# bbye98/mdhelper

Hardware: AMD Instinct MI355X
Metric: pair-distances binned/sec (higher is better)
Workload: dtype f32 filter + f64 contract arithmetic, u64 counts

## Files before the change

mdhelper_amd/csrc/mdx_rdf.hip:

```cpp

#include "mdx_common.hpp"
#include "mdx_internal.hpp"
#include "mdx_molecules.hpp"
#include "mdx_rdf_device.hpp"
#include "mdx_rdf_cell.hpp"
#include "mdx_traj.hpp"

#include <cmath>

namespace mdx {


static double thresh_ge(double e)
{
    if (!(e > 0.0))
        return 0.0;
    double t = e * e;
    while (std::sqrt(t) >= e && t > 0.0)
        t = std::nextafter(t, 0.0);
    while (std::sqrt(t) < e)
        t = std::nextafter(t, INFINITY);
    return t;
}

// ... 392 lines not shown
        if (!lazy_orig)
            MDX_TRY(h->d_po2.ensure(16 * e_p2));
        MDX_TRY(h->d_bb2.ensure(16 * e_b2));
    }
    unsigned *d_misc = h->d_misc.as<unsigned>();
    if (!tri)
        hipLaunchKernelGGL(rdf_check_boxes_kernel, dim3((unsigned)ceil_div(n_frames, 256)), dim3(256),
                           0, h->stream, d_boxes, n_frames, d_misc + 1);

    size_t base = sizeof(float4) * 256 + sizeof(double) * (h->n_bins + 1);
    const size_t lds_budget = 64 * 1024;
    const size_t lds_six_blocks = 13 * 1024;
    int n_hist = 8;
    while (n_hist > 4 && base + size_t(n_hist) * cell_hist_stride(h->n_bins) * 4 > lds_six_blocks)
        n_hist >>= 1;
    while (n_hist > 1 && base + size_t(n_hist) * cell_hist_stride(h->n_bins) * 4 > lds_budget)
        n_hist >>= 1;
    size_t lds = base + size_t(n_hist) * cell_hist_stride(h->n_bins) * 4;
    const bool gh = lds > lds_budget;
    if (gh)
        lds = sizeof(float4) * 256;
    const bool lower = h->edges.front() > 0.0;
    void (*kern)(CellArgs) = nullptr;
#define MDX_CELL_PICK(E, L)                                                                     \
    kern = tri ? (gh ? rdf_cell_pair_kernel<E, L, 1, true> : rdf_cell_pair_kernel<E, L, 0, true>) \
               : (gh ? rdf_cell_pair_kernel<E, L, 1> : rdf_cell_pair_kernel<E, L, 0>)
    if (excl && lower) MDX_CELL_PICK(true, true);
    else if (excl) MDX_CELL_PICK(true, false);
    else if (lower) MDX_CELL_PICK(false, true);
    else MDX_CELL_PICK(false, false);
#undef MDX_CELL_PICK
    if (h->occ_kernel != reinterpret_cast<const void *>(kern) || h->occ_lds != lds) {
        int per_cu = 0, cus = 0;
        MDX_HIP(hipOccupancyMaxActiveBlocksPerMultiprocessor(&per_cu, reinterpret_cast<const void *>(kern), 256, lds));
        MDX_HIP(hipDeviceGetAttribute(&cus, hipDeviceAttributeMultiprocessorCount, h->dev));
        h->occ_kernel = reinterpret_cast<const void *>(kern);
        h->occ_lds = lds;
        h->occ_blocks_per_xcd = std::max<int64_t>(1, int64_t(std::max(per_cu, 1)) * std::max(cus, 8) / 8);
    }
    const int64_t blocks_per_xcd = h->occ_blocks_per_xcd;

    hipStream_t s_sort = h->stream;
    for (int64_t f0 = 0; f0 < n_frames; f0 += slab) {
        const int64_t nf = std::min(slab, n_frames - f0);
        float4 *pw1 = h->d_pw1.as<float4>();
        float4 *po1 = lazy_orig ? nullptr : h->d_po1.as<float4>();
        float4 *bb1 = h->d_bb1.as<float4>(), *bc1 = h->d_bb16_1.as<float4>();
        float4 *pw2 = self ? pw1 : h->d_pw2.as<float4>();
        float4 *po2 = self ? po1 : (lazy_orig ? nullptr : h->d_po2.as<float4>());
// ... 796 lines not shown
```

mdhelper_amd/csrc/mdx_rdf_cell.hpp:

```cpp
#pragma once

#include "mdx_rdf_device.hpp"

struct CellArgs {
    const float4 *pw1, *po1, *bb1;
    const float4 *pw2, *po2, *bb2;
    const float4 *bb16_2;
    const float *in1, *in2;
    int n1_in, n2_in;
    const float *boxes;
    const float *tri;
    const double *thresh;
    unsigned long long *counts;
    const unsigned *maxabs_bits;
    unsigned long long *exact_counter;
    unsigned long long *tilepair_counter;
    unsigned long long *clock_counter;
    double t_lo, t_hi, r0, r1;
    int n1p, n2p;
    int n_bins, n_hist, n_rep;
    int self, frame0;
    int n_frames;
    int tags_everywhere;
    unsigned *work;
    unsigned flush_units;
    int spread;
};

constexpr unsigned CELL_WORK_STRIDE = 32;
constexpr size_t CELL_WORK_BYTES = 8 * CELL_WORK_STRIDE * 4;

constexpr int CELL_MAX = 16384;
constexpr int SORT_THREADS = 1024;
constexpr int CELL_QCAP = 1024;
constexpr int CELL_CHUNK = 1;
constexpr int CELL_NCHUNK = 64 / CELL_CHUNK;
constexpr int CELL_TODO = 128;
__host__ __device__ constexpr int cell_hist_stride(int n_bins) { return n_bins + 1; }

struct HistLdsRep {
    unsigned *h;
    int sh;
    __device__ inline void add(int k, unsigned w) const { atomicAdd(h + (k << sh), w); }
};
__device__ inline int cell_hist_shift(const HistLdsRep &h) { return h.sh; }
template <typename Hist> __device__ inline int cell_hist_shift(const Hist &) { return 0; }

struct CellGrid {
    int nc[3];
    float Lf[3];
    double Ld[3], invLd[3];
    __device__ inline void init(const float *box, int n)
    {
        double vol = 1.0;
#pragma unroll
        for (int k = 0; k < 3; ++k) {
            Lf[k] = box[k];
            Ld[k] = (double)box[k];
            invLd[k] = 1.0 / Ld[k];
            vol *= Ld[k];
        }
        const double a = cbrt(64.0 * vol / (double)max(n, 1));
        nc[0] = min(max((int)rint(Ld[0] / a), 1), 64);
        nc[1] = min(max((int)rint(Ld[1] / a), 1), 64);
        nc[2] = max((int)rint(16.0 * Ld[2] / a), 1);
        while (nc[0] * nc[1] * nc[2] > CELL_MAX)
// ... 258 lines not shown
};

__device__ inline float cell_uniform(float v)
{
    return __int_as_float(__builtin_amdgcn_readfirstlane(__float_as_int(v)));
}

__device__ inline const __constant__ CellArgs *cell_args()
{
    auto p = __builtin_amdgcn_kernarg_segment_ptr();
    asm volatile("" : "+s"(p));
    return (const __constant__ CellArgs *)p;
}

__device__ inline unsigned cell_opaque(unsigned v)
{
    v = __builtin_amdgcn_readfirstlane(v);
    asm volatile("" : "+s"(v));
    return v;
}

struct CellWave {
    uint2 *todo;
    unsigned n_todo;
    unsigned overflow;
    unsigned n_exact;
};

template <bool LOWER, int TAGS>
__device__ inline void cell_filter(const CellHot &c, float fx, float fy, float fz, int tag_i,
                                   int tag_j, float &pos, bool &cand, bool &sure)
{
    float r2 = __fmaf_rn(fz, fz, __fmaf_rn(fy, fy, fx * fx));
    pos = __fmaf_rn(__builtin_amdgcn_sqrtf(r2), c.inv_w, c.pos0);
    const float t = __builtin_amdgcn_fractf(pos);
    cand = LOWER ? (r2 < c.cand_hi && r2 >= c.cand_lo) : (r2 < c.cand_hi);
    sure = t < c.sure_w;
    if (TAGS)
        cand = cand && (tag_i != tag_j);
}

__device__ inline void cell_exact_ctx(const CellHot &c, const CellArgs &a, PairCtx<true> &cx)
{
#pragma unroll
    for (int k = 0; k < 3; ++k) {
        cx.Ld[k] = (double)c.L[k];
        cx.invd[k] = (double)c.invL[k];
    }
    cx.r0f = (float)a.r0;
    cx.inv_wf = c.inv_w;
}

template <bool LOWER, int TAGS, int MODE, typename Hist>
__device__ inline void cell_step(const CellHot &c, const CellArgs &a, const Hist &hist, float fx,
                                 float fy, float fz, int tag_i, int tag_j, unsigned i_base,
                                 unsigned j_idx, unsigned w, CellWave &wv)
{
    float r2 = __fmaf_rn(fz, fz, __fmaf_rn(fy, fy, fx * fx));
    const float pos = __fmaf_rn(__builtin_amdgcn_sqrtf(r2), c.inv_w, c.pos0);
    const float t = __builtin_amdgcn_fractf(pos);
    unsigned long long m_todo;
    if (MODE == 1) {
        bool cand = LOWER ? (r2 < c.cand_hi && r2 >= c.cand_lo) : (r2 < c.cand_hi);
        if (TAGS)
            cand = cand && (tag_i != tag_j);
        const bool sure = t < c.sure_w;
        m_todo = __builtin_amdgcn_ballot_w64(cand && !sure);
        if (cand && sure && pos < (float)a.n_bins)
            hist.add((int)pos, w);
    } else {
        const unsigned hbase = (unsigned)(size_t)(__attribute__((address_space(3))) unsigned *)hist.h;
        const int hshift = cell_hist_shift(hist) + 2;
        unsigned tmp;
        if (LOWER && TAGS)
            asm volatile("v_cmpx_gt_f32_e32 %[hi], %[r2]\n\tv_cmpx_le_f32_e32 %[lo], %[r2]\n\tv_cmpx_ne_u32_e32 %[ti], %[tj]\n\t"
                         "v_cmp_le_f32_e64 %[mt], %[sw], %[t]\n\tv_cvt_i32_f32_e32 %[tmp], %[pos]\n\t"
                         "s_andn2_b64 exec, exec, %[mt]\n\tv_lshl_add_u32 %[tmp], %[tmp], %[sh], %[hb]\n\t"
                         "ds_add_u32 %[tmp], %[w]\n\ts_mov_b64 exec, -1"
                         : [mt] "=&s"(m_todo), [tmp] "=&v"(tmp)
                         : [hi] "s"(c.cand_hi), [lo] "s"(c.cand_lo), [r2] "v"(r2), [sw] "s"(c.sure_w), [t] "v"(t),
                           [pos] "v"(pos), [hb] "v"(hbase), [w] "v"(w), [sh] "s"(hshift), [ti] "v"(tag_i), [tj] "v"(tag_j)
                         : "memory");
        else if (LOWER)
            asm volatile("v_cmpx_gt_f32_e32 %[hi], %[r2]\n\tv_cmpx_le_f32_e32 %[lo], %[r2]\n\t"
                         "v_cmp_le_f32_e64 %[mt], %[sw], %[t]\n\tv_cvt_i32_f32_e32 %[tmp], %[pos]\n\t"
                         "s_andn2_b64 exec, exec, %[mt]\n\tv_lshl_add_u32 %[tmp], %[tmp], %[sh], %[hb]\n\t"
                         "ds_add_u32 %[tmp], %[w]\n\ts_mov_b64 exec, -1"
                         : [mt] "=&s"(m_todo), [tmp] "=&v"(tmp)
                         : [hi] "s"(c.cand_hi), [lo] "s"(c.cand_lo), [r2] "v"(r2), [sw] "s"(c.sure_w), [t] "v"(t),
                           [pos] "v"(pos), [hb] "v"(hbase), [w] "v"(w), [sh] "s"(hshift)
                         : "memory");
        else if (TAGS)
            asm volatile("v_cmpx_gt_f32_e32 %[hi], %[r2]\n\tv_cmpx_ne_u32_e32 %[ti], %[tj]\n\t"
                         "v_cmp_le_f32_e64 %[mt], %[sw], %[t]\n\tv_cvt_i32_f32_e32 %[tmp], %[pos]\n\t"
                         "s_andn2_b64 exec, exec, %[mt]\n\tv_lshl_add_u32 %[tmp], %[tmp], %[sh], %[hb]\n\t"
                         "ds_add_u32 %[tmp], %[w]\n\ts_mov_b64 exec, -1"
                         : [mt] "=&s"(m_todo), [tmp] "=&v"(tmp)
                         : [hi] "s"(c.cand_hi), [r2] "v"(r2), [sw] "s"(c.sure_w), [t] "v"(t), [pos] "v"(pos),
                           [hb] "v"(hbase), [w] "v"(w), [sh] "s"(hshift), [ti] "v"(tag_i), [tj] "v"(tag_j)
                         : "memory");
        else
            asm volatile("v_cmpx_gt_f32_e32 %[hi], %[r2]\n\t"
                         "v_cmp_le_f32_e64 %[mt], %[sw], %[t]\n\tv_cvt_i32_f32_e32 %[tmp], %[pos]\n\t"
                         "s_andn2_b64 exec, exec, %[mt]\n\tv_lshl_add_u32 %[tmp], %[tmp], %[sh], %[hb]\n\t"
                         "ds_add_u32 %[tmp], %[w]\n\ts_mov_b64 exec, -1"
                         : [mt] "=&s"(m_todo), [tmp] "=&v"(tmp)
                         : [hi] "s"(c.cand_hi), [r2] "v"(r2), [sw] "s"(c.sure_w), [t] "v"(t), [pos] "v"(pos),
                           [hb] "v"(hbase), [w] "v"(w), [sh] "s"(hshift)
                         : "memory");
    }
    if (__builtin_expect(m_todo != 0ull, 0)) {
        const unsigned cnt = (unsigned)__popcll(m_todo);
        if (wv.n_todo + cnt <= (unsigned)CELL_TODO) {
            if ((m_todo >> (threadIdx.x & 63u)) & 1ull) {
                const unsigned rank = __builtin_amdgcn_mbcnt_hi(
                    (unsigned)(m_todo >> 32), __builtin_amdgcn_mbcnt_lo((unsigned)m_todo, 0u));
                wv.todo[wv.n_todo + rank] =
                    make_uint2(i_base + (threadIdx.x & 63u), j_idx);
            }
            wv.n_todo += cnt;
        } else {
            wv.overflow = 1u;
        }
    }
}

template <typename Hist>
__device__ inline void cell_flush(const CellHot &c, const CellArgs &a, const double *sT,
                                  const Hist &hist, CellWave &wv, const CellOrig &po1f,
                                  const CellOrig &po2f)
{
    __builtin_amdgcn_fence(__ATOMIC_RELEASE, "wavefront");
    __builtin_amdgcn_wave_barrier();
    __builtin_amdgcn_fence(__ATOMIC_ACQUIRE, "wavefront");
    PairCtx<true> cx;
    cell_exact_ctx(c, a, cx);
    const unsigned lane = threadIdx.x & 63u;
    for (unsigned e0 = 0; e0 < wv.n_todo; e0 += 64u) {
        if (e0 + lane < wv.n_todo) {
            const uint2 e = wv.todo[e0 + lane];
            cell_pair_exact(cx, a, sT, hist, po1f.at(e.x), po2f.at(e.y & 0x7fffffffu),
                            (e.y >> 31) + 1u, c.tri);
        }
    }
    wv.n_exact += wv.n_todo;
    wv.n_todo = 0u;
    __builtin_amdgcn_fence(__ATOMIC_RELEASE, "wavefront");
    __builtin_amdgcn_wave_barrier();
}

template <bool LOWER, bool EXCL, typename Hist>
__device__ inline void cell_slow_unit(const CellHot &c, const CellArgs &a, const double *sT,
                                      const Hist &hist, const float4 *sJw, int j0, int nj,
                                      unsigned u_mask, bool tags, int general, const float *geo,
                                      const float4 &p0, const float4 &p1, const CellOrig &po1f,
                                      const CellOrig &po2f, unsigned i_idx0, unsigned jbase,
                                      unsigned w, CellWave &wv)
{
    for (int jj = j0; jj < j0 + nj; ++jj) {
        const float4 q = sJw[jj];
        for (int u = 0; u < 2; ++u) {
            if (!((u_mask >> u) & 1u))
                continue;
            const float4 &p = u ? p1 : p0;
            float fx = q.x - p.x, fy = q.y - p.y, fz = q.z - p.z;
            if (general & 1)
                fx = fminf(fabsf(fx), c.L[0] - fabsf(fx));
            if (general & 2)
                fy = fminf(fabsf(fy), c.L[1] - fabsf(fy));
            if (general & 4)
                fz = fminf(fabsf(fz), c.L[2] - fabsf(fz));
            float pos;
            bool cand, sure;
            cell_filter<LOWER, 0>(c, fx, fy, fz, 0, 0, pos, cand, sure);
            if (EXCL && tags)
                cand = cand && (__float_as_int(p.w) != __float_as_int(q.w));
            const bool todo = cand && !sure;
            const unsigned long long m_todo = __builtin_amdgcn_ballot_w64(todo);
            if (m_todo == 0ull)
                continue;
            if (wv.n_todo > (unsigned)CELL_TODO - 64u)
                cell_flush(c, a, sT, hist, wv, po1f, po2f);
            if (todo) {
                const unsigned rank = __builtin_amdgcn_mbcnt_hi(
                    (unsigned)(m_todo >> 32), __builtin_amdgcn_mbcnt_lo((unsigned)m_todo, 0u));
                wv.todo[wv.n_todo + rank] =
                    make_uint2(i_idx0 + 64u * u, (jbase + jj) | ((w - 1u) << 31));
            }
            wv.n_todo += (unsigned)__popcll(m_todo);
        }
    }
}

template <bool EXCL, bool LOWER, int MODE, bool TRI = false>
__global__ __launch_bounds__(256, TRI ? 4 : 7) void rdf_cell_pair_kernel(CellArgs a)
{
    constexpr bool GH = MODE == 1;
    extern __shared__ __align__(16) unsigned char smem_raw[];
    float4 *sJ = reinterpret_cast<float4 *>(smem_raw);
    double *sT = reinterpret_cast<double *>(smem_raw + sizeof(float4) * 256);
    unsigned *sh = reinterpret_cast<unsigned *>(sT + (a.n_bins + 1));
    __shared__ unsigned s_exact, s_units, s_general, s_qn, s_qnext, s_next;
    __shared__ unsigned sQ[CELL_QCAP];
    __shared__ uint2 s_todo[4][CELL_TODO];
    __shared__ float s_geo[48];
    __shared__ unsigned sQimg[TRI ? CELL_QCAP : 1];

    const int tid = threadIdx.x, lane = tid & 63, wave = tid >> 6;
    long long clk0 = 0, rt0 = 0;
    if (a.clock_counter && tid == 0) {
        clk0 = clock64();
        rt0 = wall_clock64();
    }
    const int t64_2 = a.n2p / 64;

    if (!GH) {
        for (int b = tid; b <= a.n_bins; b += 256)
            sT[b] = a.thresh[b];
        for (int b = tid; b < a.n_hist * cell_hist_stride(a.n_bins); b += 256)
            sh[b] = 0u;
    }
    if (tid == 0) {
        s_exact = 0u;
        s_units = 0u;
        s_general = 0u;
        s_next = atomicAdd(a.work + CELL_WORK_STRIDE * (blockIdx.x & 7u), 1u);
    }
    __syncthreads();

    unsigned long long *out = a.counts + int64_t(blockIdx.x % unsigned(a.n_rep)) * a.n_bins;
    const double *thr = GH ? a.thresh : sT;
    const int rep_log = __builtin_amdgcn_readfirstlane(31 - __clz(a.n_hist));
    HistLdsRep hl{sh + (GH ? 0 : (lane & (a.n_hist - 1))), GH ? 0 : rep_log};
    HistGlobal hg{out};
    CellHot hot{};

    float4 *sJw = sJ + wave * 64;
    CellWave wv{s_todo[wave], 0u, 0u, 0u};
    unsigned n_units = 0, n_general = 0;
    unsigned lds_units = 0;
    for (;;) {
    const unsigned item = __builtin_amdgcn_readfirstlane(s_next);
    int frame_l, I;
    {
        const unsigned xcd = cell_opaque(blockIdx.x) & 7u;
        const auto *A = cell_args();
        const unsigned tiles = unsigned(A->n1p) >> 7;
        if (A->spread) {
            const unsigned g = item * 8u + xcd;
            if (g >= unsigned(A->n_frames) * tiles)
                break;
            const unsigned fq = __builtin_amdgcn_readfirstlane(g / tiles);
            frame_l = int(fq);
            I = int(g - fq * tiles);
        } else {
            const unsigned nfx = unsigned(A->n_frames + 7 - int(xcd)) >> 3;
            if (item >= nfx * tiles)
                break;
            const unsigned fq = __builtin_amdgcn_readfirstlane(item / tiles);
            frame_l = int(fq * 8u + xcd);
            I = int(item - fq * tiles);
// ... 21 lines not shown
            PairCtx<true> ctx;
            if (TRI) {
                const float *B = A->tri + int64_t(frame) * 9;
                float sum = 0.f;
                for (int i = 0; i < 9; ++i) {
                    s_geo[31 + i] = B[i];
                    sum += fabsf(B[i]);
                }
                const float pseudo[3] = {4.f * sum, 4.f * sum, 4.f * sum};
                ctx.init(pseudo, A->maxabs_bits, A->r0, A->r1, A->n_bins);
            } else {
                ctx.init(A->boxes + int64_t(frame) * 6, A->maxabs_bits, A->r0, A->r1, A->n_bins);
            }
            const float Lmax = fmaxf(ctx.Lf[0], fmaxf(ctx.Lf[1], ctx.Lf[2]));
            const float cut = sqrtf(ctx.cand_hi) + 1e-5f * Lmax;
            for (int k = 0; k < 3; ++k) {
                s_geo[k] = ctx.Lf[k];
                s_geo[3 + k] = ctx.invf[k];
            }
            s_geo[6] = cut;
            s_geo[7] = cut * cut;
            s_geo[26] = ctx.cand_hi;
            s_geo[27] = ctx.cand_lo;
            s_geo[28] = ctx.inv_wf;
            s_geo[29] = -ctx.r0f * ctx.inv_wf - ctx.eta;
            s_geo[30] = 1.0f - 2.0f * ctx.eta;
        }
        const float4 *BB1 = A->bb1 + int64_t(frame) * (A->n1p / 64) * 2 + int64_t(I) * 4;
        const float4 l0 = BB1[0], h0 = BB1[1], l1 = BB1[2], h1 = BB1[3];
        const float lo0[3] = {l0.x, l0.y, l0.z}, hi0[3] = {h0.x, h0.y, h0.z};
        const float lo1[3] = {l1.x, l1.y, l1.z}, hi1[3] = {h1.x, h1.y, h1.z};
        for (int k = 0; k < 3; ++k) {
            const float lo = fminf(lo0[k], lo1[k]), hi = fmaxf(hi0[k], hi1[k]);
            s_geo[8 + k] = 0.5f * (lo + hi);
            s_geo[11 + k] = 0.5f * (hi - lo);
            s_geo[14 + k] = 0.5f * (lo0[k] + hi0[k]);
            s_geo[17 + k] = 0.5f * (lo1[k] + hi1[k]);
            s_geo[20 + k] = 0.5f * (hi0[k] - lo0[k]);
            s_geo[23 + k] = 0.5f * (hi1[k] - lo1[k]);
        }
        s_qn = 0u;
        s_qnext = 0u;
    }
    float4 p0, p1;
    {
        const auto *A = cell_args();
        const float4 *PW1 = A->pw1 + int64_t(frame) * A->n1p + int64_t(I) * 128;
        int l = lane;
        asm volatile("" : "+v"(l));
// ... 176 lines not shown
                    const float hJ[3] = {0.5f * (hi.x - lo.x), 0.5f * (hi.y - lo.y), 0.5f * (hi.z - lo.z)};
                    sg2 = 0.f;
#pragma unroll
                    for (int k = 0; k < 3; ++k) {
                        float gap = fmaxf(0.f, fabsf(cJ[k] - s_geo[14 + 3 * h + k]) -
                                                   (s_geo[20 + 3 * h + k] + hJ[k]));
                        sg2 = __fmaf_rn(gap, gap, sg2);
                    }
                }
                sub = __ballot(sg2 <= s_geo[7]) & SUB_ALL;
            }
            __builtin_amdgcn_fence(__ATOMIC_RELEASE, "wavefront");
            sJw[lane] = pj;
            __builtin_amdgcn_fence(__ATOMIC_ACQUIRE, "wavefront");
            __builtin_amdgcn_wave_barrier();
            const bool diag = a.self && Jt <= 2 * I + 1;
            unsigned w = (a.self && !diag) ? 2u : 1u;
            asm volatile("" : "+v"(w));
            const unsigned jbase = unsigned(Jt) * 64u | ((a.self && !diag) ? 0x80000000u : 0u);
            const bool tags = EXCL && (a.tags_everywhere || diag);
            if (!gen) {
                const unsigned mark = wv.n_todo;
                n_units += (unsigned)__popcll(sub) + (CELL_CHUNK == 1 ? (unsigned)__popcll(sub1) : 0u);
#define MDX_CELL_HALF(TG, P, IB, Q, JJ)                                                            \
    if (GH) cell_step<LOWER, TG, MODE>(hot, a, hg, Q.x - P.x, Q.y - P.y, Q.z - P.z, __float_as_int(P.w), __float_as_int(Q.w), IB, (JJ), w, wv); \
    else cell_step<LOWER, TG, MODE>(hot, a, hl, Q.x - P.x, Q.y - P.y, Q.z - P.z, __float_as_int(P.w), __float_as_int(Q.w), IB, (JJ), w, wv);
#define MDX_CELL_UNITS_CHUNKS(TG)                                                                         \
    for (unsigned long long rem = sub; rem;) {                                                     \
        const int s = __builtin_ctzll(rem) >> 1;                                                   \
        const unsigned bits = unsigned(rem >> (2 * s)) & 3u;                                       \
        rem &= ~(3ull << (2 * s));                                                                 \
        const unsigned jg = jbase + unsigned(CELL_CHUNK * s);                                      \
        float4 q[CELL_CHUNK];                                                                      \
        _Pragma("unroll") for (int c = 0; c < CELL_CHUNK; ++c) q[c] = sJw[CELL_CHUNK * s + c];     \
               \
        if (CELL_CHUNK == 2) asm volatile("" ::"v"(q[0].w), "v"(q[1].w));                          \
        else _Pragma("unroll") for (int c = 0; c < CELL_CHUNK; ++c) asm volatile("" ::"v"(q[c].w)); \
        if (bits & 1u) {                                                                           \
            _Pragma("unroll") for (int c = 0; c < CELL_CHUNK; ++c)                                 \
            {                                                                                      \
                MDX_CELL_HALF(TG, p0, i_base0, q[c], jg + unsigned(c))                             \
            }                                                                                      \
        }                                                                                          \
        if (bits & 2u) {                                                                           \
            _Pragma("unroll") for (int c = 0; c < CELL_CHUNK; ++c)                                 \
            {                                                                                      \
                MDX_CELL_HALF(TG, p1, i_base0 + 64u, q[c], jg + unsigned(c))                       \
            }                                                                                      \
        }                                                                                          \
    }
#define MDX_CELL_ROW_LOOP(TG, MASK, BODY)                                                          \
    for (unsigned long long rem = (MASK); rem;) {                                                  \
        const int r = __builtin_ctzll(rem);                                                        \
        asm("s_bitset0_b64 %0, %1" : "+s"(rem) : "s"(r));                                          \
        const float4 q = sJw[r];                                                                   \
        asm volatile("" ::"v"(q.w));                                       \
        BODY                                                                                       \
    }
#define MDX_CELL_ROW2_LOOP(TG, MASK, BODY)                                                         \
    for (unsigned long long rem = (MASK); rem;) {                                                  \
        const int r = __builtin_ctzll(rem);                                                        \
        asm("s_bitset0_b64 %0, %1" : "+s"(rem) : "s"(r));                                          \
        const float4 q = sJw[r], q1 = sJw[r + 1];                                                  \
        asm volatile("" ::"v"(q.w), "v"(q1.w));                                                    \
        BODY                                                                                       \
    }
#define MDX_CELL_UNITS_ROWS(TG)                                                                    \
    {                                                                                              \
        const unsigned long long both = sub & sub1;                                                \
         \
        const unsigned long long pairs = both & (both >> 1) & 0x5555555555555555ull;               \
        const unsigned long long paired = pairs | (pairs << 1);                                    \
        MDX_CELL_ROW2_LOOP(TG, pairs,                                                              \
                          MDX_CELL_HALF(TG, p0, i_base0, q, jbase + unsigned(r))                   \
                          MDX_CELL_HALF(TG, p0, i_base0, q1, jbase + unsigned(r) + 1u)             \
                          MDX_CELL_HALF(TG, p1, i_base0 + 64u, q, jbase + unsigned(r))             \
                          MDX_CELL_HALF(TG, p1, i_base0 + 64u, q1, jbase + unsigned(r) + 1u))      \
        MDX_CELL_ROW_LOOP(TG, both & ~paired,                                                      \
                          MDX_CELL_HALF(TG, p0, i_base0, q, jbase + unsigned(r))                   \
                          MDX_CELL_HALF(TG, p1, i_base0 + 64u, q, jbase + unsigned(r)))            \
                                                  \
        const unsigned long long only0 = sub & ~sub1, only1 = sub1 & ~sub;                         \
        const unsigned long long pairs0 = only0 & (only0 >> 1) & 0x5555555555555555ull;            \
        const unsigned long long pairs1 = only1 & (only1 >> 1) & 0x5555555555555555ull;            \
        MDX_CELL_ROW2_LOOP(TG, pairs0,                                                             \
                          MDX_CELL_HALF(TG, p0, i_base0, q, jbase + unsigned(r))                   \
                          MDX_CELL_HALF(TG, p0, i_base0, q1, jbase + unsigned(r) + 1u))            \
        MDX_CELL_ROW2_LOOP(TG, pairs1,                                                             \
                          MDX_CELL_HALF(TG, p1, i_base0 + 64u, q, jbase + unsigned(r))             \
                          MDX_CELL_HALF(TG, p1, i_base0 + 64u, q1, jbase + unsigned(r) + 1u))      \
        MDX_CELL_ROW_LOOP(TG, only0 & ~(pairs0 | (pairs0 << 1)),                                   \
                          MDX_CELL_HALF(TG, p0, i_base0, q, jbase + unsigned(r)))                  \
        MDX_CELL_ROW_LOOP(TG, only1 & ~(pairs1 | (pairs1 << 1)),                                   \
                          MDX_CELL_HALF(TG, p1, i_base0 + 64u, q, jbase + unsigned(r)))            \
    }
#define MDX_CELL_UNITS(TG)                                                                         \
    if (CELL_CHUNK == 1) {                                                                         \
        MDX_CELL_UNITS_ROWS(TG)                                                                    \
    } else {                                                                                       \
        MDX_CELL_UNITS_CHUNKS(TG)                                                                  \
    }
                if (tags) {
                    MDX_CELL_UNITS(1)
                } else {
                    MDX_CELL_UNITS(0)
                }
#undef MDX_CELL_UNITS
#undef MDX_CELL_UNITS_ROWS
#undef MDX_CELL_ROW_LOOP
#undef MDX_CELL_ROW2_LOOP
#undef MDX_CELL_UNITS_CHUNKS
#undef MDX_CELL_HALF
                if (__builtin_expect(wv.overflow != 0u, 0)) {
                    wv.overflow = 0u;
                    wv.n_todo = mark;
                    for (unsigned long long rem = CELL_CHUNK == 1 ? (sub | sub1) : sub; rem;) {
                        const int s = CELL_CHUNK == 1 ? __builtin_ctzll(rem) : (__builtin_ctzll(rem) >> 1);
                        const unsigned bits = CELL_CHUNK == 1
                                                  ? (unsigned((sub >> s) & 1ull) | (unsigned((sub1 >> s) & 1ull) << 1))
                                                  : (unsigned(rem >> (2 * s)) & 3u);
                        rem &= CELL_CHUNK == 1 ? ~(1ull << s) : ~(3ull << (2 * s));
                        if (GH) cell_slow_unit<LOWER, EXCL>(hot, a, thr, hg, sJw, CELL_CHUNK * s, CELL_CHUNK, bits, tags, 0, s_geo, p0, p1, MDX_PO1F(), MDX_PO2(), i_idx0, jbase, w, wv);
                        else cell_slow_unit<LOWER, EXCL>(hot, a, thr, hl, sJw, CELL_CHUNK * s, CELL_CHUNK, bits, tags, 0, s_geo, p0, p1, MDX_PO1F(), MDX_PO2(), i_idx0, jbase, w, wv);
                    }
                }
            } else {
                n_units += 2 * CELL_NCHUNK;
                n_general += 2 * CELL_NCHUNK;
                const unsigned mark = wv.n_todo;
#define MDX_CELL_GENERAL(GM)                                                                       \
    _Pragma("unroll 2") for (int jj = 0; jj < 64; ++jj)                                            \
    {                                                                                              \
        float4 q = sJw[jj];                                                                        \
        asm volatile("" ::"v"(q.w));  \
        _Pragma("unroll") for (int u = 0; u < 2; ++u)                                              \
        {                                                                                          \
            const float4 &p = u ? p1 : p0;                                                         \
            float fx = q.x - p.x, fy = q.y - p.y, fz = q.z - p.z;                                  \
            if ((GM) & 1) fx = fminf(fabsf(fx), hot.L[0] - fabsf(fx));                             \
            if ((GM) & 2) fy = fminf(fabsf(fy), hot.L[1] - fabsf(fy));                             \
            if ((GM) & 4) fz = fminf(fabsf(fz), hot.L[2] - fabsf(fz));                             \
            if (GH) cell_step<LOWER, EXCL ? 1 : 0, MODE>(hot, a, hg, fx, fy, fz, __float_as_int(p.w), __float_as_int(q.w), i_base0 + 64u * u, jbase + jj, w, wv); \
            else cell_step<LOWER, EXCL ? 1 : 0, MODE>(hot, a, hl, fx, fy, fz, __float_as_int(p.w), __float_as_int(q.w), i_base0 + 64u * u, jbase + jj, w, wv); \
        }                                                                                          \
    }
                switch (gen) {
                case 1: MDX_CELL_GENERAL(1) break;
                case 2: MDX_CELL_GENERAL(2) break;
                case 3: MDX_CELL_GENERAL(3) break;
                case 4: MDX_CELL_GENERAL(4) break;
                case 5: MDX_CELL_GENERAL(5) break;
                case 6: MDX_CELL_GENERAL(6) break;
                default: MDX_CELL_GENERAL(7) break;
                }
#undef MDX_CELL_GENERAL
                if (__builtin_expect(wv.overflow != 0u, 0)) {
                    wv.overflow = 0u;
                    wv.n_todo = mark;
                    if (GH) cell_slow_unit<LOWER, EXCL>(hot, a, thr, hg, sJw, 0, 64, 3u, true, gen, s_geo, p0, p1, MDX_PO1F(), MDX_PO2(), i_idx0, jbase, w, wv);
                    else cell_slow_unit<LOWER, EXCL>(hot, a, thr, hl, sJw, 0, 64, 3u, true, gen, s_geo, p0, p1, MDX_PO1F(), MDX_PO2(), i_idx0, jbase, w, wv);
                }
            }
            if (wv.n_todo >= 64u) {
                if (GH) cell_flush(hot, a, thr, hg, wv, MDX_PO1F(), MDX_PO2());
                else cell_flush(hot, a, thr, hl, wv, MDX_PO1F(), MDX_PO2());
            }
            }
        }
        if (round0 + CELL_QCAP >= t64_2 && wv.n_todo) {
            if (GH) cell_flush(hot, a, thr, hg, wv, MDX_PO1F(), MDX_PO2());
            else cell_flush(hot, a, thr, hl, wv, MDX_PO1F(), MDX_PO2());
        }
        __syncthreads();
    }
    }
#undef MDX_PO1F
#undef MDX_PO2
    }
    if (lane == 0) {
        if (wv.n_exact) atomicAdd(&s_exact, wv.n_exact);
        if (n_units) atomicAdd(&s_units, n_units);
        if (n_general) atomicAdd(&s_general, n_general);
    }
    __syncthreads();
    if (tid == 0) {
        const unsigned so = rdf_stat_offset(blockIdx.x);
        if (s_exact) atomicAdd(a.exact_counter + so, (unsigned long long)s_exact);
        if (s_units) atomicAdd(a.tilepair_counter + so, (unsigned long long)s_units);
        if (s_general) atomicAdd(a.tilepair_counter + so + 1, (unsigned long long)s_general);
        if (a.clock_counter) {
            atomicAdd(a.clock_counter + so, (unsigned long long)(clock64() - clk0));
            atomicAdd(a.clock_counter + so + 1, (unsigned long long)(wall_clock64() - rt0));
        }
    }
// ... 11 lines not shown
```

Measured before the change: 2118 billion.

## Add fixed-point bin mode and move todo-queue append into inline asm slow path

Adds a MODE==2 kernel variant, used when LDS histograms are used and there are at most 254 bins. It scales the bin position by 2^16 and converts it to u32, so the integer bin is the high 16 bits and the fractional 'sure' test becomes a 16-bit integer compare. This replaces fract plus float compare with cvt_u32, cmp_u16 and mad_u32_u16, with a bias applied to the histogram base. The todo-queue append for ambiguous pairs also moves into the inline asm as an out-of-line subsection branch, which removes the ballot and popcount C++ path from the hot loop. Both changes aim to cut VALU and SALU instructions per pair, at the cost of more complex asm and some precision-handling risk near bin edges.

```diff
diff --git a/mdhelper_amd/csrc/mdx_rdf.hip b/mdhelper_amd/csrc/mdx_rdf.hip
--- a/mdhelper_amd/csrc/mdx_rdf.hip
+++ b/mdhelper_amd/csrc/mdx_rdf.hip
@@ -438,9 +438,14 @@
         lds = sizeof(float4) * 256;
     const bool lower = h->edges.front() > 0.0;
     void (*kern)(CellArgs) = nullptr;
+    bool fxp = !gh && h->n_bins + 2 <= 256;
+    if (const char *e = getenv("MDX_RDF_CELL_FIXED"))
+        fxp = fxp && atoi(e) != 0;
 #define MDX_CELL_PICK(E, L)                                                                     \
-    kern = tri ? (gh ? rdf_cell_pair_kernel<E, L, 1, true> : rdf_cell_pair_kernel<E, L, 0, true>) \
-               : (gh ? rdf_cell_pair_kernel<E, L, 1> : rdf_cell_pair_kernel<E, L, 0>)
+    kern = tri ? (gh ? rdf_cell_pair_kernel<E, L, 1, true>                                      \
+                     : fxp ? rdf_cell_pair_kernel<E, L, 2, true> : rdf_cell_pair_kernel<E, L, 0, true>) \
+               : (gh ? rdf_cell_pair_kernel<E, L, 1>                                            \
+                     : fxp ? rdf_cell_pair_kernel<E, L, 2> : rdf_cell_pair_kernel<E, L, 0>)
     if (excl && lower) MDX_CELL_PICK(true, true);
     else if (excl) MDX_CELL_PICK(true, false);
     else if (lower) MDX_CELL_PICK(false, true);
diff --git a/mdhelper_amd/csrc/mdx_rdf_cell.hpp b/mdhelper_amd/csrc/mdx_rdf_cell.hpp
--- a/mdhelper_amd/csrc/mdx_rdf_cell.hpp
+++ b/mdhelper_amd/csrc/mdx_rdf_cell.hpp
@@ -41,7 +41,8 @@
 struct HistLdsRep {
     unsigned *h;
     int sh;
-    __device__ inline void add(int k, unsigned w) const { atomicAdd(h + (k << sh), w); }
+    int bias;
+    __device__ inline void add(int k, unsigned w) const { atomicAdd(h + ((k + bias) << sh), w); }
 };
 __device__ inline int cell_hist_shift(const HistLdsRep &h) { return h.sh; }
 template <typename Hist> __device__ inline int cell_hist_shift(const Hist &) { return 0; }
@@ -346,24 +347,35 @@
 
 struct CellWave {
     uint2 *todo;
+    unsigned todo_lds;
     unsigned n_todo;
     unsigned overflow;
     unsigned n_exact;
 };
 
-template <bool LOWER, int TAGS>
+__device__ inline unsigned cell_fx_u32(float P)
+{
+    unsigned u;
+    asm("v_cvt_u32_f32_e32 %0, %1" : "=v"(u) : "v"(P));
+    return u;
+}
+
+template <bool LOWER, int TAGS, bool FX>
 __device__ inline void cell_filter(const CellHot &c, float fx, float fy, float fz, int tag_i,
-                                   int tag_j, float &pos, bool &cand, bool &sure)
+                                   int tag_j, bool &cand, bool &sure)
 {
     float r2 = __fmaf_rn(fz, fz, __fmaf_rn(fy, fy, fx * fx));
-    pos = __fmaf_rn(__builtin_amdgcn_sqrtf(r2), c.inv_w, c.pos0);
-    const float t = __builtin_amdgcn_fractf(pos);
+    const float pos = __fmaf_rn(__builtin_amdgcn_sqrtf(r2), c.inv_w, c.pos0);
     cand = LOWER ? (r2 < c.cand_hi && r2 >= c.cand_lo) : (r2 < c.cand_hi);
-    sure = t < c.sure_w;
+    if (FX)
+        sure = (cell_fx_u32(pos) & 0xffffu) < __float_as_uint(c.sure_w);
+    else
+        sure = __builtin_amdgcn_fractf(pos) < c.sure_w;
     if (TAGS)
         cand = cand && (tag_i != tag_j);
 }
 
+template <bool FX>
 __device__ inline void cell_exact_ctx(const CellHot &c, const CellArgs &a, PairCtx<true> &cx)
 {
 #pragma unroll
@@ -372,84 +384,98 @@
         cx.invd[k] = (double)c.invL[k];
     }
     cx.r0f = (float)a.r0;
-    cx.inv_wf = c.inv_w;
-}
-
-template <bool LOWER, int TAGS, int MODE, typename Hist>
+    cx.inv_wf = FX ? c.inv_w * 0x1p-16f : c.inv_w;
+}
+
+#define MDX_STEP_PRE_00 "v_cmpx_gt_f32_e32 %[hi], %[r2]\n\t"
+#define MDX_STEP_PRE_10 MDX_STEP_PRE_00 "v_cmpx_le_f32_e32 %[lo], %[r2]\n\t"
+#define MDX_STEP_PRE_01 MDX_STEP_PRE_00 "v_cmpx_ne_u32_e32 %[ti], %[tj]\n\t"
+#define MDX_STEP_PRE_11 MDX_STEP_PRE_10 "v_cmpx_ne_u32_e32 %[ti], %[tj]\n\t"
+#define MDX_STEP_BIN_FLOAT                                                                         \
+    "v_cmp_le_f32_e32 vcc, %[sw], %[y]\n\tv_cvt_i32_f32_e32 %[tmp], %[x]\n\t"                      \
+    "s_andn2_b64 exec, exec, vcc\n\tv_lshl_add_u32 %[tmp], %[tmp], %[sh], %[hb]\n\t"
+#define MDX_STEP_BIN_FX                                                                            \
+    "v_cvt_u32_f32_e32 %[y], %[x]\n\tv_cmp_le_u16_e32 vcc, %[sw], %[y]\n\t"                        \
+    "v_mad_u32_u16 %[tmp], %[y], %[sh], %[hb] op_sel:[1,0,0,0]\n\ts_andn2_b64 exec, exec, vcc\n\t"
+#define MDX_STEP_TAIL                                                                              \
+    "ds_add_u32 %[tmp], %[w]\n\ts_mov_b64 exec, -1\n\ts_cbranch_vccnz .Lmdx_todo_%=\n"             \
+    ".Lmdx_back_%=:\n\t.subsection 1\n"                                                            \
+    ".Lmdx_todo_%=:\n\ts_bcnt1_i32_b64 %[st], vcc\n\ts_add_u32 %[st], %[st], %[nt]\n\t"            \
+    "s_cmp_gt_u32 %[st], %[cap]\n\ts_cbranch_scc1 .Lmdx_full_%=\n\t"                               \
+    "v_mbcnt_lo_u32_b32 %[y], vcc_lo, 0\n\tv_mbcnt_hi_u32_b32 %[y], vcc_hi, %[y]\n\t"              \
+    "v_add_u32_e32 %[y], %[nt], %[y]\n\tv_lshl_add_u32 %[y], %[y], 3, %[td]\n\t"                   \
+    "v_mbcnt_lo_u32_b32 %[tmp], -1, 0\n\tv_mbcnt_hi_u32_b32 %[tmp], -1, %[tmp]\n\t"                \
+    "v_add_u32_e32 %[tmp], %[ib], %[tmp]\n\tv_mov_b32_e32 %[x], %[jb]\n\t"                         \
+    "v_add_u32_e32 %[x], %[jr], %[x]\n\tv_add_u32_e32 %[x], %[jo], %[x]\n\t"                       \
+    "s_mov_b64 exec, vcc\n\tds_write2_b32 %[y], %[tmp], %[x] offset1:1\n\t"                        \
+    "s_mov_b64 exec, -1\n\ts_mov_b32 %[nt], %[st]\n\ts_branch .Lmdx_back_%=\n"                     \
+    ".Lmdx_full_%=:\n\ts_mov_b32 %[ov], 1\n\ts_branch .Lmdx_back_%=\n\t.subsection 0\n\t"
+template <bool LOWER, int TAGS, int MODE, int JO = 0, typename Hist>
 __device__ inline void cell_step(const CellHot &c, const CellArgs &a, const Hist &hist, float fx,
                                  float fy, float fz, int tag_i, int tag_j, unsigned i_base,
-                                 unsigned j_idx, unsigned w, CellWave &wv)
+                                 unsigned jbase, unsigned jr, unsigned w, CellWave &wv)
 {
     float r2 = __fmaf_rn(fz, fz, __fmaf_rn(fy, fy, fx * fx));
-    const float pos = __fmaf_rn(__builtin_amdgcn_sqrtf(r2), c.inv_w, c.pos0);
-    const float t = __builtin_amdgcn_fractf(pos);
-    unsigned long long m_todo;
+    float pos = __fmaf_rn(__builtin_amdgcn_sqrtf(r2), c.inv_w, c.pos0);
     if (MODE == 1) {
+        const float t = __builtin_amdgcn_fractf(pos);
         bool cand = LOWER ? (r2 < c.cand_hi && r2 >= c.cand_lo) : (r2 < c.cand_hi);
         if (TAGS)
             cand = cand && (tag_i != tag_j);
         const bool sure = t < c.sure_w;
-        m_todo = __builtin_amdgcn_ballot_w64(cand && !sure);
+        const unsigned long long m_todo = __builtin_amdgcn_ballot_w64(cand && !sure);
         if (cand && sure && pos < (float)a.n_bins)
             hist.add((int)pos, w);
+        if (__builtin_expect(m_todo != 0ull, 0)) {
+            const unsigned cnt = (unsigned)__popcll(m_todo);
+            if (wv.n_todo + cnt <= (unsigned)CELL_TODO) {
+                if ((m_todo >> (threadIdx.x & 63u)) & 1ull) {
+                    const unsigned rank = __builtin_amdgcn_mbcnt_hi(
+                        (unsigned)(m_todo >> 32), __builtin_amdgcn_mbcnt_lo((unsigned)m_todo, 0u));
+                    wv.todo[wv.n_todo + rank] = make_uint2(i_base + (threadIdx.x & 63u), jbase + jr + unsigned(JO));
+                }
+                wv.n_todo += cnt;
+            } else {
+                wv.overflow = 1u;
+            }
+        }
     } else {
+        constexpr bool FX = MODE == 2;
         const unsigned hbase = (unsigned)(size_t)(__attribute__((address_space(3))) unsigned *)hist.h;
-        const int hshift = cell_hist_shift(hist) + 2;
-        unsigned tmp;
-        if (LOWER && TAGS)
-            asm volatile("v_cmpx_gt_f32_e32 %[hi], %[r2]\n\tv_cmpx_le_f32_e32 %[lo], %[r2]\n\tv_cmpx_ne_u32_e32 %[ti], %[tj]\n\t"
-                         "v_cmp_le_f32_e64 %[mt], %[sw], %[t]\n\tv_cvt_i32_f32_e32 %[tmp], %[pos]\n\t"
-                         "s_andn2_b64 exec, exec, %[mt]\n\tv_lshl_add_u32 %[tmp], %[tmp], %[sh], %[hb]\n\t"
-                         "ds_add_u32 %[tmp], %[w]\n\ts_mov_b64 exec, -1"
-                         : [mt] "=&s"(m_todo), [tmp] "=&v"(tmp)
-                         : [hi] "s"(c.cand_hi), [lo] "s"(c.cand_lo), [r2] "v"(r2), [sw] "s"(c.sure_w), [t] "v"(t),
-                           [pos] "v"(pos), [hb] "v"(hbase), [w] "v"(w), [sh] "s"(hshift), [ti] "v"(tag_i), [tj] "v"(tag_j)
-                         : "memory");
-        else if (LOWER)
-            asm volatile("v_cmpx_gt_f32_e32 %[hi], %[r2]\n\tv_cmpx_le_f32_e32 %[lo], %[r2]\n\t"
-                         "v_cmp_le_f32_e64 %[mt], %[sw], %[t]\n\tv_cvt_i32_f32_e32 %[tmp], %[pos]\n\t"
-                         "s_andn2_b64 exec, exec, %[mt]\n\tv_lshl_add_u32 %[tmp], %[tmp], %[sh], %[hb]\n\t"
-                         "ds_add_u32 %[tmp], %[w]\n\ts_mov_b64 exec, -1"
-                         : [mt] "=&s"(m_todo), [tmp] "=&v"(tmp)
-                         : [hi] "s"(c.cand_hi), [lo] "s"(c.cand_lo), [r2] "v"(r2), [sw] "s"(c.sure_w), [t] "v"(t),
-                           [pos] "v"(pos), [hb] "v"(hbase), [w] "v"(w), [sh] "s"(hshift)
-                         : "memory");
-        else if (TAGS)
-            asm volatile("v_cmpx_gt_f32_e32 %[hi], %[r2]\n\tv_cmpx_ne_u32_e32 %[ti], %[tj]\n\t"
-                         "v_cmp_le_f32_e64 %[mt], %[sw], %[t]\n\tv_cvt_i32_f32_e32 %[tmp], %[pos]\n\t"
-                         "s_andn2_b64 exec, exec, %[mt]\n\tv_lshl_add_u32 %[tmp], %[tmp], %[sh], %[hb]\n\t"
-                         "ds_add_u32 %[tmp], %[w]\n\ts_mov_b64 exec, -1"
-                         : [mt] "=&s"(m_todo), [tmp] "=&v"(tmp)
-                         : [hi] "s"(c.cand_hi), [r2] "v"(r2), [sw] "s"(c.sure_w), [t] "v"(t), [pos] "v"(pos),
-                           [hb] "v"(hbase), [w] "v"(w), [sh] "s"(hshift), [ti] "v"(tag_i), [tj] "v"(tag_j)
-                         : "memory");
+        const int hsh = cell_hist_shift(hist) + 2;
+        const unsigned sh = FX ? (1u << hsh) : unsigned(hsh);
+        float y;
+        if (FX)
+            asm volatile("" : "=v"(y));
         else
-            asm volatile("v_cmpx_gt_f32_e32 %[hi], %[r2]\n\t"
-                         "v_cmp_le_f32_e64 %[mt], %[sw], %[t]\n\tv_cvt_i32_f32_e32 %[tmp], %[pos]\n\t"
-                         "s_andn2_b64 exec, exec, %[mt]\n\tv_lshl_add_u32 %[tmp], %[tmp], %[sh], %[hb]\n\t"
-                         "ds_add_u32 %[tmp], %[w]\n\ts_mov_b64 exec, -1"
-                         : [mt] "=&s"(m_todo), [tmp] "=&v"(tmp)
-                         : [hi] "s"(c.cand_hi), [r2] "v"(r2), [sw] "s"(c.sure_w), [t] "v"(t), [pos] "v"(pos),
-                           [hb] "v"(hbase), [w] "v"(w), [sh] "s"(hshift)
-                         : "memory");
-    }
-    if (__builtin_expect(m_todo != 0ull, 0)) {
-        const unsigned cnt = (unsigned)__popcll(m_todo);
-        if (wv.n_todo + cnt <= (unsigned)CELL_TODO) {
-            if ((m_todo >> (threadIdx.x & 63u)) & 1ull) {
-                const unsigned rank = __builtin_amdgcn_mbcnt_hi(
-                    (unsigned)(m_todo >> 32), __builtin_amdgcn_mbcnt_lo((unsigned)m_todo, 0u));
-                wv.todo[wv.n_todo + rank] =
-                    make_uint2(i_base + (threadIdx.x & 63u), j_idx);
-            }
-            wv.n_todo += cnt;
+            y = __builtin_amdgcn_fractf(pos);
+        unsigned tmp, st;
+#define MDX_STEP_ASM(PRE, BIN)                                                                     \
+    asm volatile(PRE BIN MDX_STEP_TAIL                                                             \
+                 : [x] "+v"(pos), [y] "+v"(y), [tmp] "=&v"(tmp), [st] "=&s"(st), [nt] "+s"(wv.n_todo),   \
+                   [ov] "+s"(wv.overflow)                                                           \
+                 : [hi] "s"(c.cand_hi), [lo] "s"(LOWER ? c.cand_lo : c.cand_hi), [r2] "v"(r2),     \
+                   [sw] "s"(c.sure_w), [hb] "v"(hbase), [w] "v"(w), [sh] "s"(sh),                  \
+                   [ti] "v"(TAGS ? tag_i : __float_as_int(r2)), [tj] "v"(TAGS ? tag_j : __float_as_int(r2)), \
+                   [td] "s"(wv.todo_lds), [ib] "s"(i_base), [jb] "s"(jbase), [jr] "s"(jr),          \
+                   [jo] "i"(JO), [cap] "i"(CELL_TODO)                                               \
+                 : "memory", "vcc", "scc")
+        if (FX) {
+            if (LOWER && TAGS) MDX_STEP_ASM(MDX_STEP_PRE_11, MDX_STEP_BIN_FX);
+            else if (LOWER) MDX_STEP_ASM(MDX_STEP_PRE_10, MDX_STEP_BIN_FX);
+            else if (TAGS) MDX_STEP_ASM(MDX_STEP_PRE_01, MDX_STEP_BIN_FX);
+            else MDX_STEP_ASM(MDX_STEP_PRE_00, MDX_STEP_BIN_FX);
         } else {
-            wv.overflow = 1u;
-        }
-    }
-}
-
-template <typename Hist>
+            if (LOWER && TAGS) MDX_STEP_ASM(MDX_STEP_PRE_11, MDX_STEP_BIN_FLOAT);
+            else if (LOWER) MDX_STEP_ASM(MDX_STEP_PRE_10, MDX_STEP_BIN_FLOAT);
+            else if (TAGS) MDX_STEP_ASM(MDX_STEP_PRE_01, MDX_STEP_BIN_FLOAT);
+            else MDX_STEP_ASM(MDX_STEP_PRE_00, MDX_STEP_BIN_FLOAT);
+        }
+#undef MDX_STEP_ASM
+    }
+}
+
+template <bool FX, typename Hist>
 __device__ inline void cell_flush(const CellHot &c, const CellArgs &a, const double *sT,
                                   const Hist &hist, CellWave &wv, const CellOrig &po1f,
                                   const CellOrig &po2f)
@@ -458,7 +484,7 @@
     __builtin_amdgcn_wave_barrier();
     __builtin_amdgcn_fence(__ATOMIC_ACQUIRE, "wavefront");
     PairCtx<true> cx;
-    cell_exact_ctx(c, a, cx);
+    cell_exact_ctx<FX>(c, a, cx);
     const unsigned lane = threadIdx.x & 63u;
     for (unsigned e0 = 0; e0 < wv.n_todo; e0 += 64u) {
         if (e0 + lane < wv.n_todo) {
@@ -473,7 +499,7 @@
     __builtin_amdgcn_wave_barrier();
 }
 
-template <bool LOWER, bool EXCL, typename Hist>
+template <bool LOWER, bool EXCL, bool FX, typename Hist>
 __device__ inline void cell_slow_unit(const CellHot &c, const CellArgs &a, const double *sT,
                                       const Hist &hist, const float4 *sJw, int j0, int nj,
                                       unsigned u_mask, bool tags, int general, const float *geo,
@@ -494,9 +520,8 @@
                 fy = fminf(fabsf(fy), c.L[1] - fabsf(fy));
             if (general & 4)
                 fz = fminf(fabsf(fz), c.L[2] - fabsf(fz));
-            float pos;
             bool cand, sure;
-            cell_filter<LOWER, 0>(c, fx, fy, fz, 0, 0, pos, cand, sure);
+            cell_filter<LOWER, 0, FX>(c, fx, fy, fz, 0, 0, cand, sure);
             if (EXCL && tags)
                 cand = cand && (__float_as_int(p.w) != __float_as_int(q.w));
             const bool todo = cand && !sure;
@@ -504,7 +529,7 @@
             if (m_todo == 0ull)
                 continue;
             if (wv.n_todo > (unsigned)CELL_TODO - 64u)
-                cell_flush(c, a, sT, hist, wv, po1f, po2f);
+                cell_flush<FX>(c, a, sT, hist, wv, po1f, po2f);
             if (todo) {
                 const unsigned rank = __builtin_amdgcn_mbcnt_hi(
                     (unsigned)(m_todo >> 32), __builtin_amdgcn_mbcnt_lo((unsigned)m_todo, 0u));
@@ -520,6 +545,7 @@
 __global__ __launch_bounds__(256, TRI ? 4 : 7) void rdf_cell_pair_kernel(CellArgs a)
 {
     constexpr bool GH = MODE == 1;
+    constexpr bool FX = MODE == 2;
     extern __shared__ __align__(16) unsigned char smem_raw[];
     float4 *sJ = reinterpret_cast<float4 *>(smem_raw);
     double *sT = reinterpret_cast<double *>(smem_raw + sizeof(float4) * 256);
@@ -555,12 +581,15 @@
     unsigned long long *out = a.counts + int64_t(blockIdx.x % unsigned(a.n_rep)) * a.n_bins;
     const double *thr = GH ? a.thresh : sT;
     const int rep_log = __builtin_amdgcn_readfirstlane(31 - __clz(a.n_hist));
-    HistLdsRep hl{sh + (GH ? 0 : (lane & (a.n_hist - 1))), GH ? 0 : rep_log};
+    HistLdsRep hl{sh + (GH ? 0 : (lane & (a.n_hist - 1))) - (FX ? a.n_hist : 0), GH ? 0 : rep_log, FX ? 1 : 0};
     HistGlobal hg{out};
     CellHot hot{};
 
     float4 *sJw = sJ + wave * 64;
-    CellWave wv{s_todo[wave], 0u, 0u, 0u};
+    CellWave wv{s_todo[wave],
+                (unsigned)__builtin_amdgcn_readfirstlane(
+                    (int)(unsigned)(size_t)(__attribute__((address_space(3))) uint2 *)s_todo[wave]),
+                0u, 0u, 0u};
     unsigned n_units = 0, n_general = 0;
     unsigned lds_units = 0;
     for (;;) {
@@ -628,9 +657,16 @@
             s_geo[7] = cut * cut;
             s_geo[26] = ctx.cand_hi;
             s_geo[27] = ctx.cand_lo;
-            s_geo[28] = ctx.inv_wf;
-            s_geo[29] = -ctx.r0f * ctx.inv_wf - ctx.eta;
-            s_geo[30] = 1.0f - 2.0f * ctx.eta;
+            if (FX) {
+                s_geo[28] = ctx.inv_wf * 0x1p16f;
+                s_geo[29] = (float)((1.0 - A->r0 * (double)ctx.inv_wf - (double)ctx.eta) * 0x1p16);
+                const double t16 = floor((1.0 - 2.0 * (double)ctx.eta) * 0x1p16) - 1.0;
+                s_geo[30] = __uint_as_float((unsigned)fmin(fmax(t16, 0.0), 65535.0));
+            } else {
+                s_geo[28] = ctx.inv_wf;
+                s_geo[29] = -ctx.r0f * ctx.inv_wf - ctx.eta;
+                s_geo[30] = 1.0f - 2.0f * ctx.eta;
+            }
         }
         const float4 *BB1 = A->bb1 + int64_t(frame) * (A->n1p / 64) * 2 + int64_t(I) * 4;
         const float4 l0 = BB1[0], h0 = BB1[1], l1 = BB1[2], h1 = BB1[3];
@@ -853,15 +889,15 @@
             if (!gen) {
                 const unsigned mark = wv.n_todo;
                 n_units += (unsigned)__popcll(sub) + (CELL_CHUNK == 1 ? (unsigned)__popcll(sub1) : 0u);
-#define MDX_CELL_HALF(TG, P, IB, Q, JJ)                                                            \
-    if (GH) cell_step<LOWER, TG, MODE>(hot, a, hg, Q.x - P.x, Q.y - P.y, Q.z - P.z, __float_as_int(P.w), __float_as_int(Q.w), IB, (JJ), w, wv); \
-    else cell_step<LOWER, TG, MODE>(hot, a, hl, Q.x - P.x, Q.y - P.y, Q.z - P.z, __float_as_int(P.w), __float_as_int(Q.w), IB, (JJ), w, wv);
+#define MDX_CELL_HALF(TG, P, IB, Q, JR, JO)                                                        \
+    if (GH) cell_step<LOWER, TG, MODE, JO>(hot, a, hg, Q.x - P.x, Q.y - P.y, Q.z - P.z, __float_as_int(P.w), __float_as_int(Q.w), IB, jbase, (JR), w, wv); \
+    else cell_step<LOWER, TG, MODE, JO>(hot, a, hl, Q.x - P.x, Q.y - P.y, Q.z - P.z, __float_as_int(P.w), __float_as_int(Q.w), IB, jbase, (JR), w, wv);
 #define MDX_CELL_UNITS_CHUNKS(TG)                                                                         \
     for (unsigned long long rem = sub; rem;) {                                                     \
         const int s = __builtin_ctzll(rem) >> 1;                                                   \
         const unsigned bits = unsigned(rem >> (2 * s)) & 3u;                                       \
         rem &= ~(3ull << (2 * s));                                                                 \
-        const unsigned jg = jbase + unsigned(CELL_CHUNK * s);                                      \
+        const unsigned jg = unsigned(CELL_CHUNK * s);                                              \
         float4 q[CELL_CHUNK];                                                                      \
         _Pragma("unroll") for (int c = 0; c < CELL_CHUNK; ++c) q[c] = sJw[CELL_CHUNK * s + c];     \
                \
@@ -870,13 +906,13 @@
         if (bits & 1u) {                                                                           \
             _Pragma("unroll") for (int c = 0; c < CELL_CHUNK; ++c)                                 \
             {                                                                                      \
-                MDX_CELL_HALF(TG, p0, i_base0, q[c], jg + unsigned(c))                             \
+                MDX_CELL_HALF(TG, p0, i_base0, q[c], jg + unsigned(c), 0)                             \
             }                                                                                      \
         }                                                                                          \
         if (bits & 2u) {                                                                           \
             _Pragma("unroll") for (int c = 0; c < CELL_CHUNK; ++c)                                 \
             {                                                                                      \
-                MDX_CELL_HALF(TG, p1, i_base0 + 64u, q[c], jg + unsigned(c))                       \
+                MDX_CELL_HALF(TG, p1, i_base0 + 64u, q[c], jg + unsigned(c), 0)                       \
             }                                                                                      \
         }                                                                                          \
     }
@@ -903,27 +939,27 @@
         const unsigned long long pairs = both & (both >> 1) & 0x5555555555555555ull;               \
         const unsigned long long paired = pairs | (pairs << 1);                                    \
         MDX_CELL_ROW2_LOOP(TG, pairs,                                                              \
-                          MDX_CELL_HALF(TG, p0, i_base0, q, jbase + unsigned(r))                   \
-                          MDX_CELL_HALF(TG, p0, i_base0, q1, jbase + unsigned(r) + 1u)             \
-                          MDX_CELL_HALF(TG, p1, i_base0 + 64u, q, jbase + unsigned(r))             \
-                          MDX_CELL_HALF(TG, p1, i_base0 + 64u, q1, jbase + unsigned(r) + 1u))      \
+                          MDX_CELL_HALF(TG, p0, i_base0, q, unsigned(r), 0)                   \
+                          MDX_CELL_HALF(TG, p0, i_base0, q1, unsigned(r), 1)             \
+                          MDX_CELL_HALF(TG, p1, i_base0 + 64u, q, unsigned(r), 0)             \
+                          MDX_CELL_HALF(TG, p1, i_base0 + 64u, q1, unsigned(r), 1))      \
         MDX_CELL_ROW_LOOP(TG, both & ~paired,                                                      \
-                          MDX_CELL_HALF(TG, p0, i_base0, q, jbase + unsigned(r))                   \
-                          MDX_CELL_HALF(TG, p1, i_base0 + 64u, q, jbase + unsigned(r)))            \
+                          MDX_CELL_HALF(TG, p0, i_base0, q, unsigned(r), 0)                   \
+                          MDX_CELL_HALF(TG, p1, i_base0 + 64u, q, unsigned(r), 0))            \
                                                   \
         const unsigned long long only0 = sub & ~sub1, only1 = sub1 & ~sub;                         \
         const unsigned long long pairs0 = only0 & (only0 >> 1) & 0x5555555555555555ull;            \
         const unsigned long long pairs1 = only1 & (only1 >> 1) & 0x5555555555555555ull;            \
         MDX_CELL_ROW2_LOOP(TG, pairs0,                                                             \
-                          MDX_CELL_HALF(TG, p0, i_base0, q, jbase + unsigned(r))                   \
-                          MDX_CELL_HALF(TG, p0, i_base0, q1, jbase + unsigned(r) + 1u))            \
+                          MDX_CELL_HALF(TG, p0, i_base0, q, unsigned(r), 0)                   \
+                          MDX_CELL_HALF(TG, p0, i_base0, q1, unsigned(r), 1))            \
         MDX_CELL_ROW2_LOOP(TG, pairs1,                                                             \
-                          MDX_CELL_HALF(TG, p1, i_base0 + 64u, q, jbase + unsigned(r))             \
-                          MDX_CELL_HALF(TG, p1, i_base0 + 64u, q1, jbase + unsigned(r) + 1u))      \
+                          MDX_CELL_HALF(TG, p1, i_base0 + 64u, q, unsigned(r), 0)             \
+                          MDX_CELL_HALF(TG, p1, i_base0 + 64u, q1, unsigned(r), 1))      \
         MDX_CELL_ROW_LOOP(TG, only0 & ~(pairs0 | (pairs0 << 1)),                                   \
-                          MDX_CELL_HALF(TG, p0, i_base0, q, jbase + unsigned(r)))                  \
+                          MDX_CELL_HALF(TG, p0, i_base0, q, unsigned(r), 0))                  \
         MDX_CELL_ROW_LOOP(TG, only1 & ~(pairs1 | (pairs1 << 1)),                                   \
-                          MDX_CELL_HALF(TG, p1, i_base0 + 64u, q, jbase + unsigned(r)))            \
+                          MDX_CELL_HALF(TG, p1, i_base0 + 64u, q, unsigned(r), 0))            \
     }
 #define MDX_CELL_UNITS(TG)                                                                         \
     if (CELL_CHUNK == 1) {                                                                         \
@@ -951,8 +987,8 @@
                                                   ? (unsigned((sub >> s) & 1ull) | (unsigned((sub1 >> s) & 1ull) << 1))
                                                   : (unsigned(rem >> (2 * s)) & 3u);
                         rem &= CELL_CHUNK == 1 ? ~(1ull << s) : ~(3ull << (2 * s));
-                        if (GH) cell_slow_unit<LOWER, EXCL>(hot, a, thr, hg, sJw, CELL_CHUNK * s, CELL_CHUNK, bits, tags, 0, s_geo, p0, p1, MDX_PO1F(), MDX_PO2(), i_idx0, jbase, w, wv);
-                        else cell_slow_unit<LOWER, EXCL>(hot, a, thr, hl, sJw, CELL_CHUNK * s, CELL_CHUNK, bits, tags, 0, s_geo, p0, p1, MDX_PO1F(), MDX_PO2(), i_idx0, jbase, w, wv);
+                        if (GH) cell_slow_unit<LOWER, EXCL, FX>(hot, a, thr, hg, sJw, CELL_CHUNK * s, CELL_CHUNK, bits, tags, 0, s_geo, p0, p1, MDX_PO1F(), MDX_PO2(), i_idx0, jbase, w, wv);
+                        else cell_slow_unit<LOWER, EXCL, FX>(hot, a, thr, hl, sJw, CELL_CHUNK * s, CELL_CHUNK, bits, tags, 0, s_geo, p0, p1, MDX_PO1F(), MDX_PO2(), i_idx0, jbase, w, wv);
                     }
                 }
             } else {
@@ -971,8 +1007,8 @@
             if ((GM) & 1) fx = fminf(fabsf(fx), hot.L[0] - fabsf(fx));                             \
             if ((GM) & 2) fy = fminf(fabsf(fy), hot.L[1] - fabsf(fy));                             \
             if ((GM) & 4) fz = fminf(fabsf(fz), hot.L[2] - fabsf(fz));                             \
-            if (GH) cell_step<LOWER, EXCL ? 1 : 0, MODE>(hot, a, hg, fx, fy, fz, __float_as_int(p.w), __float_as_int(q.w), i_base0 + 64u * u, jbase + jj, w, wv); \
-            else cell_step<LOWER, EXCL ? 1 : 0, MODE>(hot, a, hl, fx, fy, fz, __float_as_int(p.w), __float_as_int(q.w), i_base0 + 64u * u, jbase + jj, w, wv); \
+            if (GH) cell_step<LOWER, EXCL ? 1 : 0, MODE>(hot, a, hg, fx, fy, fz, __float_as_int(p.w), __float_as_int(q.w), i_base0 + 64u * u, jbase, unsigned(jj), w, wv); \
+            else cell_step<LOWER, EXCL ? 1 : 0, MODE>(hot, a, hl, fx, fy, fz, __float_as_int(p.w), __float_as_int(q.w), i_base0 + 64u * u, jbase, unsigned(jj), w, wv); \
         }                                                                                          \
     }
                 switch (gen) {
@@ -988,19 +1024,19 @@
                 if (__builtin_expect(wv.overflow != 0u, 0)) {
                     wv.overflow = 0u;
                     wv.n_todo = mark;
-                    if (GH) cell_slow_unit<LOWER, EXCL>(hot, a, thr, hg, sJw, 0, 64, 3u, true, gen, s_geo, p0, p1, MDX_PO1F(), MDX_PO2(), i_idx0, jbase, w, wv);
-                    else cell_slow_unit<LOWER, EXCL>(hot, a, thr, hl, sJw, 0, 64, 3u, true, gen, s_geo, p0, p1, MDX_PO1F(), MDX_PO2(), i_idx0, jbase, w, wv);
+                    if (GH) cell_slow_unit<LOWER, EXCL, FX>(hot, a, thr, hg, sJw, 0, 64, 3u, true, gen, s_geo, p0, p1, MDX_PO1F(), MDX_PO2(), i_idx0, jbase, w, wv);
+                    else cell_slow_unit<LOWER, EXCL, FX>(hot, a, thr, hl, sJw, 0, 64, 3u, true, gen, s_geo, p0, p1, MDX_PO1F(), MDX_PO2(), i_idx0, jbase, w, wv);
                 }
             }
             if (wv.n_todo >= 64u) {
-                if (GH) cell_flush(hot, a, thr, hg, wv, MDX_PO1F(), MDX_PO2());
-                else cell_flush(hot, a, thr, hl, wv, MDX_PO1F(), MDX_PO2());
+                if (GH) cell_flush<FX>(hot, a, thr, hg, wv, MDX_PO1F(), MDX_PO2());
+                else cell_flush<FX>(hot, a, thr, hl, wv, MDX_PO1F(), MDX_PO2());
             }
             }
         }
         if (round0 + CELL_QCAP >= t64_2 && wv.n_todo) {
-            if (GH) cell_flush(hot, a, thr, hg, wv, MDX_PO1F(), MDX_PO2());
-            else cell_flush(hot, a, thr, hl, wv, MDX_PO1F(), MDX_PO2());
+            if (GH) cell_flush<FX>(hot, a, thr, hg, wv, MDX_PO1F(), MDX_PO2());
+            else cell_flush<FX>(hot, a, thr, hl, wv, MDX_PO1F(), MDX_PO2());
         }
         __syncthreads();
     }
```

Result: no change. 2109 billion (-0.4%).
